# mikkleini/slam.net

Hardware: AMD Instinct MI355X
Metric: candidate-pose distance evals/sec on 2048^2 map, 1080-ray scan, 1/2/4/8 GPU (higher is better)
Workload: dtype f32 transform + u16 gather / integer sum

## Files before the change

include/slamhip.h:

```cpp
#ifndef SLAMHIP_H
#define SLAMHIP_H

#include <stddef.h>
#include <stdint.h>

#ifdef __cplusplus
extern "C" {
#endif

#define SLAMHIP_OK            0
#define SLAMHIP_ERR_INVALID  (-1)
#define SLAMHIP_ERR_HIP      (-2)
#define SLAMHIP_ERR_NOMEM    (-3)
#define SLAMHIP_ERR_STATE    (-4)
#define SLAMHIP_ERR_RCCL     (-5)
#define SLAMHIP_ERR_TIMEOUT  (-6)

typedef struct slamhip_ctx    slamhip_ctx;
typedef struct slamhip_cs     slamhip_cs;
typedef struct slamhip_csproc slamhip_csproc;
typedef struct slamhip_hs     slamhip_hs;
typedef struct slamhip_hsproc slamhip_hsproc;
typedef struct slamhip_group  slamhip_group;
typedef struct slamhip_comm   slamhip_comm;
// ... 69 lines not shown
                                      int32_t count, uint64_t *d_out_key);
int32_t slamhip_cs_search_shard_enqueue(slamhip_cs *cs, const float search_pose[3], int32_t first, int32_t count,
                                        const uint64_t **d_key);
int32_t slamhip_cs_key_read(slamhip_cs *cs, const uint64_t *d_key, uint64_t *out_key);
int32_t slamhip_cs_pose_from_key(slamhip_cs *cs, const float search_pose[3], uint64_t key,
                                 float out_pose[3], int32_t *out_dist, int32_t *out_index);

int32_t slamhip_cs_update_holemap(slamhip_cs *cs, const float pose[3], float hole_width, int32_t quality);
int32_t slamhip_cs_update_holemap_pxcs(slamhip_cs *cs, const float pxcs[4], float hole_width, int32_t quality);
int32_t slamhip_cs_update_obstaclemap(slamhip_cs *cs, const float pose[3], int32_t max_obstacle_hits);
int32_t slamhip_cs_update_obstaclemap_pxcs(slamhip_cs *cs, const float pxcs[4], int32_t max_obstacle_hits);
int32_t slamhip_cs_last_holemap_pixels(slamhip_cs *cs, int64_t *out_pixels);
int32_t slamhip_cs_maps_checksum(slamhip_cs *cs, uint64_t out[2]);

int32_t slamhip_cs_selfcheck_failures(slamhip_cs *cs, uint32_t *out_failures);

int32_t slamhip_cs_prelaunch_stats(slamhip_cs *cs, uint64_t out[4]);

int32_t slamhip_cs_plan_stats(slamhip_cs *cs, uint64_t out[4]);

int32_t slamhip_cs_search_and_update(slamhip_cs *cs, const float search_pose[3], float hole_width,
                                     int32_t quality, int32_t max_obstacle_hits, float out_pose[3],
                                     int32_t *out_dist, int32_t *out_index);
int32_t slamhip_cs_scan_search_and_update(slamhip_cs *cs, const float *xy, int32_t n_points, const float search_pose[3], float hole_width,
                                          int32_t quality, int32_t max_obstacle_hits, float out_pose[3], int32_t *out_dist,
                                          int32_t *out_index);
int32_t slamhip_cs_search_and_update_pxcs(slamhip_cs *cs, const float *pxcs_search, const float *pxcs_update_hole,
                                          const float *pxcs_update_obstacle, int32_t K,
                                          float hole_width, int32_t quality, int32_t max_obstacle_hits,
                                          int32_t *out_index, int32_t *out_dist);
// ... 147 lines not shown
```

slam.net_amd/capi.py:

```python
import ctypes as C
import os
import re

import numpy as np

_HERE = os.path.dirname(os.path.abspath(__file__))
SO_PATH = os.path.join(_HERE, "libslamhip.so")
HEADER = os.path.join(os.path.dirname(_HERE), "include", "slamhip.h")

OK = 0
ERR_INVALID, ERR_HIP, ERR_NOMEM, ERR_STATE, ERR_RCCL, ERR_TIMEOUT = -1, -2, -3, -4, -5, -6
K_CS_PREP, K_CS_DISTANCE, K_CS_REDUCE, K_CS_HOLEMAP, K_CS_OBSTACLE, K_HS_MATCH, K_HS_UPDATE = range(7)

CELL_DTYPE = np.dtype([("update_index", np.int32), ("value", np.float32)])


class MatchReport(C.Structure):
    _fields_ = [("pose_map", C.c_float * 3), ("H", C.c_float * 9), ("dTr", C.c_float * 3), ("residual", C.c_float),
                ("n_in_map", C.c_int32), ("n_points", C.c_int32), ("level", C.c_int32)]


REPORT_DTYPE = np.dtype([("pose_map", np.float32, 3), ("H", np.float32, (3, 3)), ("dTr", np.float32, 3),
                         ("residual", np.float32), ("n_in_map", np.int32), ("n_points", np.int32), ("level", np.int32)])
assert C.sizeof(MatchReport) == REPORT_DTYPE.itemsize == 76
# ... 92 lines not shown
        "slamhip_cs_update_holemap": (i32, [vp, fp, f, i32]),
        "slamhip_cs_update_holemap_pxcs": (i32, [vp, fp, f, i32]),
        "slamhip_cs_update_obstaclemap": (i32, [vp, fp, i32]),
        "slamhip_cs_update_obstaclemap_pxcs": (i32, [vp, fp, i32]),
        "slamhip_cs_last_holemap_pixels": (i32, [vp, P(i64)]),
        "slamhip_cs_maps_checksum": (i32, [vp, P(u64)]),
        "slamhip_cs_search_and_update": (i32, [vp, fp, f, i32, i32, fp, ip, ip]),
        "slamhip_cs_scan_search_and_update": (i32, [vp, fp, i32, fp, f, i32, i32, fp, ip, ip]),
        "slamhip_cs_search_and_update_pxcs": (i32, [vp, fp, fp, fp, i32, f, i32, i32, ip, ip]),
        "slamhip_cs_update_maps_pxcs": (i32, [vp, fp, fp, f, i32, i32]),
        "slamhip_cs_search_report": (i32, [vp, fp, i32, fp, srp]),
        "slamhip_cs_search_distances": (i32, [vp, ip, i32]),
        "slamhip_cs_search_and_update_report": (i32, [vp, fp, i32, f, i32, i32, fp, srp]),
        "slamhip_cs_scan_search_and_update_report": (i32, [vp, fp, i32, fp, i32, f, i32, i32, fp, srp]),
        "slamhip_cs_selfcheck_failures": (i32, [vp, P(C.c_uint32)]),
        "slamhip_cs_prelaunch_stats": (i32, [vp, P(C.c_uint64)]),
        "slamhip_cs_plan_stats": (i32, [vp, P(C.c_uint64)]),
        "slamhip_cs_prepared_lists": (i32, [vp, P(C.c_uint64), P(C.c_uint64)]),
        "slamhip_csproc_create": (i32, [vp, f, i32, i32, fp, f, f, i32, i32, vpp]),
        "slamhip_csproc_destroy": (i32, [vp]),
        "slamhip_csproc_reset": (i32, [vp]),
        "slamhip_csproc_update": (i32, [vp, fp, ip, i32, fp]),
        "slamhip_csproc_get_pose": (i32, [vp, fp]),
        "slamhip_csproc_set_params": (i32, [vp, i32, f, i32, i32, i32]),
        "slamhip_csproc_set_seed": (i32, [vp, u64]),
        "slamhip_csproc_set_lattice": (i32, [vp, i32]),
        "slamhip_csproc_set_offsets": (i32, [vp, fp, i32]),
        "slamhip_csproc_set_search_report": (i32, [vp, i32, i32]),
        "slamhip_csproc_get_report": (i32, [vp, srp, ip]),
        "slamhip_csproc_cs": (i32, [vp, vpp]),
# ... 98 lines not shown
```

slam.net_amd/coreslam.py:

```python
import ctypes as C

import numpy as np

from . import capi


class Context:

    def __init__(self, device=0):
        self._h = C.c_void_p()
        capi.call("slamhip_ctx_create", int(device), C.byref(self._h))

    def close(self):
        if self._h:
            capi.lib().slamhip_ctx_destroy(self._h)
            self._h = C.c_void_p()

    @property
    def stream(self):
        return capi.lib().slamhip_ctx_stream(self._h)

    def synchronize(self):
        capi.call("slamhip_ctx_synchronize", self._h)

# ... 232 lines not shown
        v = (C.c_uint64 * 4)()
        capi.call("slamhip_cs_prelaunch_stats", self._h, v)
        return tuple(int(x) for x in v)

    @property
    def plan_stats(self):
        v = (C.c_uint64 * 4)()
        capi.call("slamhip_cs_plan_stats", self._h, v)
        return tuple(int(x) for x in v)

    @property
    def selfcheck_failures(self):
        v = C.c_uint32()
        capi.call("slamhip_cs_selfcheck_failures", self._h, C.byref(v))
        return v.value

    def search_and_update(self, search_pose, hole_width=0.6, quality=50, max_hits=10):
        sp = capi.f32(search_pose)
        pose = np.empty(3, np.float32); d, i = C.c_int32(), C.c_int32()
        capi.call("slamhip_cs_search_and_update", self._h, capi.fptr(sp), C.c_float(hole_width), int(quality),
                  int(max_hits), capi.fptr(pose), C.byref(d), C.byref(i))
        return pose, d.value, i.value


    def scan_search_and_update(self, xy, search_pose, hole_width=0.6, quality=50, max_hits=10):
        pts = np.ascontiguousarray(xy, np.float32).reshape(-1, 2)
        sp = capi.f32(search_pose)
        pose = np.empty(3, np.float32); d, i = C.c_int32(), C.c_int32()
        capi.call("slamhip_cs_scan_search_and_update", self._h, capi.fptr(pts), int(pts.shape[0]), capi.fptr(sp), C.c_float(hole_width), int(quality),
                  int(max_hits), capi.fptr(pose), C.byref(d), C.byref(i))
# ... 145 lines not shown
```

slam.net_amd/csrc/coreslam.hip:

```cpp
#include "cs_internal.h"
#include "det_trig.h"
#include "obstacle_dev.h"
#include <algorithm>
#include <numeric>
#include <math.h>
#include <stdlib.h>

__global__ void k_fill_u16(uint16_t *p, size_t n, uint16_t v)
{
    size_t i = (size_t)blockIdx.x * blockDim.x + threadIdx.x;
    const size_t stride = (size_t)gridDim.x * blockDim.x;
    for (; i < n; i += stride) p[i] = v;
}

__global__ void k_pack_holemap(const uint16_t *__restrict__ pix, uint8_t *__restrict__ out, size_t n_bytes)
{
    size_t i = (size_t)blockIdx.x * blockDim.x + threadIdx.x;
    if (i >= n_bytes) return;
    out[i] = (uint8_t)(((pix[i * 2] >> 12) << 4) | (pix[i * 2 + 1] >> 12));
}

__device__ static inline void philox4x32_10(uint32_t c[4], uint32_t k0, uint32_t k1)
{
    for (int r = 0; r < 10; r++) {
// ... 1372 lines not shown
extern "C" int32_t slamhip_cs_plan_stats(slamhip_cs *cs, uint64_t out[4])
{
    SH_CHECK_ARG(cs && out);
    for (int k = 0; k < 4; k++) out[k] = cs->plan_stats[k];
    return SLAMHIP_OK;
}

extern "C" int32_t slamhip_cs_selfcheck_failures(slamhip_cs *cs, uint32_t *out)
{
    SH_CHECK_ARG(cs && out);
    SH_HIP(hipSetDevice(cs->ctx->device));
    unsigned int *h = (unsigned int *)(cs->h_key + 8);
    SH_HIP(hipMemcpyAsync(h, cs->d_verify, sizeof(unsigned int) * 8, hipMemcpyDeviceToHost, cs->ctx->stream));
    SH_HIP(hipStreamSynchronize(cs->ctx->stream));
    *out = h[0];
    return SLAMHIP_OK;
}

extern "C" int32_t slamhip_cs_update_maps_pxcs(slamhip_cs *cs, const float pxcs_hole[4], const float pxcs_obstacle[4], float hole_width,
                                               int32_t quality, int32_t max_obstacle_hits)
{
    SH_CHECK_ARG(cs && pxcs_hole && quality >= 0 && quality <= 256 && max_obstacle_hits >= -128 && max_obstacle_hits <= 127);
    SH_HIP(hipSetDevice(cs->ctx->device));
    cs->last_hole_pixels = 0; cs->hole_pixels_pending = false;
    if (cs->n_points <= 0) return SLAMHIP_OK;
    SH_TRY(cs_launch_holemap_update(cs, nullptr, make_float4(pxcs_hole[0], pxcs_hole[1], pxcs_hole[2], pxcs_hole[3]), make_float4(0, 0, 0, 0), hole_width, quality));
    if (pxcs_obstacle)
        SH_TRY(cs_launch_obstacle_update(cs, nullptr, make_float4(pxcs_obstacle[0], pxcs_obstacle[1], pxcs_obstacle[2], pxcs_obstacle[3]), max_obstacle_hits));
    return finish_holemap(cs);
}
// ... 303 lines not shown
```

slam.net_amd/csrc/cs_internal.h:

```cpp
#pragma once
#include "common.h"
#include <time.h>
#include <stdio.h>
#include <stdlib.h>
#include <vector>
#include <utility>

#define CS_RB_MAX 64
#define CS_RB_EXTENT_PX 128.0f
#define K1_GROUP 1024
#define K1_GROUP_BIG 2048
#define K1_RING_SLOTS 4
#define K1_GROUP_SMALL 512
#define K1_PLAN_SLOTS 8


struct k1_block_term { double a, b, m, n, nr; };

struct slamhip_cs {
    slamhip_ctx *ctx;
    float physical;
    int hs; float hscale;
    int os; float oscale;
    uint16_t *d_hole;
    int8_t *d_obst;

    int n_points, cap_points;
    void *d_scan_blob, *h_scan_blob;
    char *d_scan_cur; size_t scan_blob_bytes; int scan_buf;
// ... 178 lines not shown
```

slam.net_amd/csrc/distance.hip:

```cpp
#include "cs_internal.h"
#include "det_trig.h"
#include <stdlib.h>
#include <algorithm>

#define K1_THREADS 256

__device__ static inline void k1_coords(const float4 q, const float2 p, float &fx, float &fy)
{
    fx = q.x + q.z * p.x;  fx = fx - q.w * p.y;
    fy = q.y + q.w * p.x;  fy = fy + q.z * p.y;
}

template <bool SAFE>
__device__ static inline void k1_gather_global(const uint16_t *__restrict__ map, int S, const float4 q, const float2 p,
                                               uint32_t &sum, uint32_t &cnt)
{
    float fx, fy;
    k1_coords(q, p, fx, fy);
    int ix, iy;
    if (SAFE) { ix = sh_f2i(fx); iy = sh_f2i(fy); }
    else      { ix = (int)fx;    iy = (int)fy; }
    const bool ok = ((unsigned)ix < (unsigned)S) & ((unsigned)iy < (unsigned)S);
    uint32_t v = 0;
    if (ok) v = map[(size_t)iy * S + ix];
// ... 105 lines not shown
        }
        __syncthreads();
    }
    if (w == 0) {
        for (int off = 32; off > 0; off >>= 1) {
            const unsigned long long o = __shfl_down(key, off, 64);
            key = o < key ? o : key;
        }
        if (lane == 0 && key != ~0ull) atomicMin(key_out, key);
    }
}

#define K1_KIND_SHARED 1
#define K1_KIND_GLOBAL 2
#define K1_KIND_BAND 3
#define K1_MAXP 16
#define K1_MAXR 512
#define K1_MAXBANDS 4
#define K1_MAXSTEPS (K1_MAXP * K1_MAXBANDS * 2)
static_assert(K1_MAXBANDS == 4, "the step threads split t into (piece, band) with shifts");
#define K1_TABLE_G 64
#define K1_TABLE_WGS 2048
#define K1_MAXCUT 596
#define K1_ACC_INMAP 36
#define K1_ACC_ARRIVED 50
#define K1_ZERO_OFS 0
#define K1_TILE_OFS 16

struct k1_args {
    const uint16_t *map; int S;
// ... 31 lines not shown
        unsigned short nbp;
        unsigned short first, nc;
    } tab[K1_TABLE_G];
    alignas(4) unsigned char wg_pos[K1_TABLE_WGS];
    alignas(4) unsigned short cut[K1_MAXCUT];
};
static_assert(sizeof(k1_args) <= 4096, "kernel arguments are limited to 4 KB");
static_assert(sizeof(k1_args::tab_rec) == 8 && offsetof(k1_args, tab) % 8 == 0, "table records are 8-byte aligned");
#define K1_PLAN_STEPS 15
#define K1_PLAN_REC_WORDS 128

#ifdef K1_TIMES
__device__ unsigned long long g_k1_times[4096 * 16];
__device__ unsigned long long g_k1_wstart[4096 * 16];
__device__ unsigned long long g_k1_sub[4096 * 8];
#define K1_SUB(k, v) { if (threadIdx.x == 0 && blockIdx.x < 4096) g_k1_sub[blockIdx.x * 8 + (k)] += (v); }
#define K1_STAMP(k) { if (threadIdx.x == 0 && blockIdx.x < 4096) g_k1_times[blockIdx.x * 16 + (k)] = wall_clock64(); }
#else
#define K1_STAMP(k) {}
#endif

__device__ static inline unsigned k1_tile_addr(int ix, int iy, int pitch2, int kofs)
{
    unsigned t, a;
    asm("v_lshl_add_u32 %0, %1, 1, %2" : "=v"(t) : "v"(ix), "s"(kofs));
    asm("v_mad_u32_u24 %0, %1, %2, %3" : "=v"(a) : "v"(iy), "s"(pitch2), "v"(t));
    return a;
}
__device__ static inline float k1_den(int v) { return __uint_as_float(v < 0 ? (0x80000000u | (unsigned)(-v)) : (unsigned)v); }
__device__ static inline unsigned k1_tile_addr_d(float fx, float fy, float two_d, float pitch2_d, float c_d)
{
    const float g = fmaf(truncf(fy), pitch2_d, fmaf(truncf(fx), two_d, c_d));
    return __float_as_uint(g);
}
typedef __attribute__((address_space(3))) const uint16_t k1_lds_u16;
__device__ static inline uint32_t k1_lds_load(unsigned addr) { return *(k1_lds_u16 *)(size_t)addr; }
typedef __attribute__((address_space(3))) const float k1_lds_f;
__device__ static inline float2 k1_point_lds(unsigned lds_addr)
{
    k1_lds_f *p = (k1_lds_f *)(size_t)lds_addr;
    return make_float2(p[0], p[1]);
}

typedef float k1_f32x4a8 __attribute__((ext_vector_type(4), aligned(8)));
__device__ static inline float4 k1_points2_lds(unsigned lds_addr)
{
    const k1_f32x4a8 v = *(__attribute__((address_space(3))) const k1_f32x4a8 *)(size_t)lds_addr;
    return make_float4(v.x, v.y, v.z, v.w);
// ... 138 lines not shown

    const uint16_t *__restrict__ map = a.map;
    const int S = a.S, count = a.count;
    const int t = threadIdx.x, lane = t & 63;
    int zv;
    asm volatile("v_mov_b32 %0, 0" : "=v"(zv));
    const int wv = __builtin_amdgcn_readfirstlane(t >> 6);
    const k1_wg_t W = k1_wg_decode(a, (int)blockIdx.x);
    const int g = W.g, nc = W.nc, nbp = W.nbp;
    if (a.ring_reset && blockIdx.x == 0 && t == 0)
        __hip_atomic_store(a.ring_reset, ~0ull, __ATOMIC_RELAXED, __HIP_MEMORY_SCOPE_AGENT);
    if (a.started && blockIdx.x == 0 && t == 0)
        __hip_atomic_store(a.started, a.launch_no, __ATOMIC_RELAXED, __HIP_MEMORY_SCOPE_SYSTEM);
    K1_STAMP(0)
#ifdef K1_TIMES
    if (t == 0 && blockIdx.x < 4096) { for (int k = 0; k < 8; k++) g_k1_sub[blockIdx.x * 8 + k] = 0; }
    if (t == 0 && blockIdx.x < 4096) { for (int k = 10; k < 16; k++) g_k1_times[blockIdx.x * 16 + k] = 0; g_k1_times[blockIdx.x * 16 + 14] = (unsigned long long)g; g_k1_times[blockIdx.x * 16 + 15] = (unsigned long long)nc; }
    if (lane == 0 && blockIdx.x < 4096) g_k1_wstart[blockIdx.x * 16 + (wv & 15)] = wall_clock64();
    if (t == 0 && blockIdx.x < 4096) {
        unsigned hw, xcc;
        asm volatile("s_getreg_b32 %0, hwreg(HW_REG_HW_ID)" : "=s"(hw));
        asm volatile("s_getreg_b32 %0, hwreg(HW_REG_XCC_ID)" : "=s"(xcc));
        g_k1_wstart[blockIdx.x * 16 + 15] = ((unsigned long long)(xcc & 15u) << 16) | ((hw >> 8) & 0xffu);
    }
#endif
    const int bp = W.bp, rlo = W.rlo, rhi = W.rhi;
    const int nrays = rhi - rlo;
    if (a.scan_flag) {
        uint32_t v = 0;
        if (wv == 0) {
            int spins = 0;
// ... 221 lines not shown
            const unsigned long long ts1 = wall_clock64();
            if (s > 0) K1_SUB(0, ts1 - ts0)
#endif
            const int4 ca = *(const int4 *)&stepbuf[s * 8], cb = *(const int4 *)&stepbuf[s * 8 + 4];
            {
                const int sn = s + 1 < nsteps ? s + 1 : s;
                K1_PREFETCH(sn, s + 1 < nsteps)
            }
#ifdef K1_TIMES
            const unsigned long long ts2 = wall_clock64();
            K1_SUB(1, ts2 - ts1) K1_SUB(3, 1ull)
#endif
            const int kind = __builtin_amdgcn_readfirstlane(cb.y);
            const int nr = __builtin_amdgcn_readfirstlane(cb.z) >> 16;
#ifdef K1_TIMES
            if (t == 0 && blockIdx.x < 4096) g_k1_times[blockIdx.x * 16 + 10 + kind] += (unsigned long long)nr;
            if (t == 0 && blockIdx.x < 4096 && s < 3)
                g_k1_sub[blockIdx.x * 8 + 5 + s] = (unsigned long long)kind | ((unsigned long long)__builtin_amdgcn_readfirstlane(ca.z) << 4) | ((unsigned long long)__builtin_amdgcn_readfirstlane(ca.w) << 16) | ((unsigned long long)nr << 32);
#endif
            const unsigned pbase = cpts_lds + (unsigned)zv + (unsigned)(__builtin_amdgcn_readfirstlane(cb.z) & 0xffff) * 8u;
            const int x0a = __builtin_amdgcn_readfirstlane(ca.x), y0 = __builtin_amdgcn_readfirstlane(ca.y);
            const int w8 = __builtin_amdgcn_readfirstlane(ca.z), h = __builtin_amdgcn_readfirstlane(ca.w);
            const int pitch2 = w8 << 1;
            const int kofs = (int)smem_lds + K1_TILE_OFS - ((y0 * w8 + x0a) << 1);
            const unsigned zaddr = smem_lds + K1_ZERO_OFS + (unsigned)zv;
            const bool daddr = !a.noden && (unsigned)S * (unsigned)pitch2 + 2u * (unsigned)S + (1u << 18) < (1u << 23);
            float two_v, p2d_v, cd_v;
            {
                const float two_s = k1_den(2), p2d_s = k1_den(pitch2), cd_s = k1_den(kofs);
                asm volatile("v_mov_b32 %0, %1" : "=v"(two_v) : "s"(two_s));
                asm volatile("v_mov_b32 %0, %1" : "=v"(p2d_v) : "s"(p2d_s));
                asm volatile("v_mov_b32 %0, %1" : "=v"(cd_v) : "s"(cd_s));
            }
            if (K1_EXP == 2 || K1_EXP == 3) { sum[0] += (uint32_t)nr; continue; }
            if (kind != K1_KIND_GLOBAL) {
                const bool checked = kind == K1_KIND_BAND;
                uint32_t va[CPL], vb[CPL];
                int r = 0;
                float4 pn = k1_points2_lds(pbase);
                float2 pa_n = make_float2(pn.x, pn.y), pb_n = make_float2(pn.z, pn.w);
#pragma unroll
                for (int k = 0; k < CPL; k++) { va[k] = k1_lds_load(zaddr); vb[k] = k1_lds_load(zaddr); }
                __builtin_amdgcn_sched_barrier(0);
                if (!checked && daddr) {
#define K1_DPAIR(P, NEXTREAD)                                                                       \
                    {                                                                               \
                        unsigned ada[CPL], adb[CPL];                                                \
                        float cxa_ = 0.f, sya_ = 0.f, sxa_ = 0.f, cya_ = 0.f, cxb_ = 0.f, syb_ = 0.f, sxb_ = 0.f, cyb_ = 0.f; \
                        if (LAT) {                                                                  \
                            cxa_ = q[0].z * (P).x; sya_ = q[0].w * (P).y; sxa_ = q[0].w * (P).x; cya_ = q[0].z * (P).y; \
// ... 107 lines not shown
                        k1_coords(q[k], pa, fx, fy);
                        const int ix = (int)fx, iy = (int)fy;
                        const bool ok = ((unsigned)(ix - x0a) < (unsigned)w8) & ((unsigned)(iy - y0) < (unsigned)h);
                        if (VERIFY) {
                            if (!ok && !checked) atomicAdd(a.verify, 1u);
                            if (ok && map[(size_t)iy * S + ix] != *(const uint16_t *)(smem + (k1_tile_addr(ix, iy, pitch2, kofs) - smem_lds))) atomicAdd(a.verify, 1u);
                        }
                        sum[k] += k1_lds_load(ok ? k1_tile_addr(ix, iy, pitch2, kofs) : zaddr);
                        if (checked) cnt[k] += ok ? 1u : 0u;
                    }
                }
#pragma unroll
                for (int k = 0; k < CPL; k++) sum[k] += va[k] + vb[k];
                if (VERIFY && t == 0) atomicAdd(a.verify + (checked ? 4 : 1), (unsigned)(nr * 4));
            } else {
                int r = 0;
                for (; r + 1 < nr; r += 2) {
                    const float2 pa = k1_point_lds(pbase + r * 8), pb = k1_point_lds(pbase + r * 8 + 8);
                    uint32_t ga[CPL], gb[CPL]; bool oka[CPL], okb[CPL];
#pragma unroll
                    for (int k = 0; k < CPL; k++) {
                        float fxa, fya, fxb, fyb;
                        k1_coords(q[k], pa, fxa, fya);
                        k1_coords(q[k], pb, fxb, fyb);
                        const int ixa = (int)fxa, iya = (int)fya, ixb = (int)fxb, iyb = (int)fyb;
                        oka[k] = ((unsigned)ixa < (unsigned)S) & ((unsigned)iya < (unsigned)S);
                        okb[k] = ((unsigned)ixb < (unsigned)S) & ((unsigned)iyb < (unsigned)S);
                        ga[k] = map[oka[k] ? (size_t)iya * S + ixa : 0];
                        gb[k] = map[okb[k] ? (size_t)iyb * S + ixb : 0];
                    }
#pragma unroll
                    for (int k = 0; k < CPL; k++) {
                        sum[k] += (oka[k] ? ga[k] : 0u) + (okb[k] ? gb[k] : 0u);
                        cnt[k] += (oka[k] ? 1u : 0u) + (okb[k] ? 1u : 0u);
                    }
                }
                if (r < nr) {
                    const float2 pa = k1_point_lds(pbase + r * 8);
#pragma unroll
                    for (int k = 0; k < CPL; k++) k1_gather_global<false>(map, S, q[k], pa, sum[k], cnt[k]);
                }
                if (VERIFY && t == 0) atomicAdd(a.verify + 3, (unsigned)(nr * 4));
            }
#ifdef K1_TIMES
            K1_SUB(2, wall_clock64() - ts2)
#endif
        }
#ifdef K1_TIMES
        K1_SUB(4, clock64() - sclk0)
#endif
#undef K1_PREFETCH
    }
    K1_STAMP(7)

    typedef unsigned long long u64;
    if (K1_EXP == 4) { if (sum[0] == 0x12345u && cnt[0] == 77u) a.verify[0] = 1u; return; }
    u64 *acc = a.acc + (size_t)g * GROUP + (size_t)t;
    u64 tot[CPL];
#pragma unroll
    for (int k = 0; k < CPL; k++) {
// ... 153 lines not shown

static int32_t ensure_partial(slamhip_cs *cs, size_t bytes)
{
    if (bytes <= cs->cap_partial) return SLAMHIP_OK;
    if (cs->d_partial) (void)hipFree(cs->d_partial);
    cs->d_partial = nullptr; cs->cap_partial = 0;
    bytes += bytes / 4;
    SH_HIP(hipMalloc(&cs->d_partial, bytes));
    cs->cap_partial = bytes;
    return SLAMHIP_OK;
}

constexpr int K1_BAND_PARTS = 2;
constexpr float K1_BAND_STAGE = 5.0f;
constexpr double K1_CUT_CAND = 0.9;
constexpr double K1_FBAND = 1.9, K1_FGLOBAL = 3.0;
constexpr double K1_STEPCOST = 8.0;
constexpr double K1_TAILW = 1.5;

static bool k1_chunks_legal(const slamhip_cs *cs, int nc)
{
    const int R = cs->n_points, n_rb = cs->n_rb;
    const int *rb = cs->h_rb_start.data();
    if (nc < 1 || nc > R) return false;
    int b = 0;
    const int dq = R / nc, dr = R % nc;
    int rlo = 0, rem = 0;
    for (int c = 0; c < nc; c++) {
        int rhi = rlo + dq;
        rem += dr;
        if (rem >= nc) { rem -= nc; rhi++; }
// ... 697 lines not shown
            (void)hipMemcpyFromSymbol(sb.data(), HIP_SYMBOL(g_k1_sub), sizeof(unsigned long long) * sb.size());
            double a0 = 0, a1 = 0, a2 = 0, a3 = 0, mhz = 0; int nm_ = 0;
            for (int i = 0; i < nw; i++) {
                a0 += (double)sb[i * 8] * 0.01; a1 += (double)sb[i * 8 + 1] * 0.01; a2 += (double)sb[i * 8 + 2] * 0.01; a3 += (double)sb[i * 8 + 3];
                const double comp = (double)(h[i * 16 + 7] - h[i * 16 + 6]) * 0.01;
                if (comp > 1.0) { mhz += (double)sb[i * 8 + 4] / (comp + (double)(h[i * 16 + 6] - h[i * 16 + 5]) * 0.01); nm_++; }
            }
            fprintf(stderr, "[k1 times] compute phase, mean per WG: steps %.2f | restaging %.2f us | prefetch issue %.2f us | gather loops %.2f us | shader clock ~%.0f MHz (steps incl. first staging)\n",
                    a3 / nw, a0 / nw, a1 / nw, a2 / nw, nm_ ? mhz / nm_ : 0.0);
            for (int oi = 0; oi < nw; oi += nw / 24 > 0 ? nw / 24 : 1) {
                const int i = order[(size_t)oi];
                fprintf(stderr, "  wg %4d g %2d: steps %d restaging %5.2f prefetch %5.2f loops %5.2f | rays shared %d global %d band %d\n", i, (int)h[i * 16 + 14], (int)sb[i * 8 + 3],
                        (double)sb[i * 8] * 0.01, (double)sb[i * 8 + 1] * 0.01, (double)sb[i * 8 + 2] * 0.01, (int)h[i * 16 + 11], (int)h[i * 16 + 12], (int)h[i * 16 + 13]);
            }
        }
        for (int g = 0; g < n_groups; g++) {
            double cs_ = 0, cm = 0; int n = 0; long long k4[4] = { 0, 0, 0, 0 };
            for (int i = 0; i < nw; i++) if ((int)h[i * 16 + 14] == g) {
                const double c = (double)(h[i * 16 + 7] - h[i * 16 + 6]) * 0.01;
                cs_ += c; cm = std::max(cm, c); n++;
                for (int k = 0; k < 4; k++) k4[k] += (long long)h[i * 16 + 10 + k];
            }
            fprintf(stderr, "  group %2d: chunks %2d | ray-steps own %lld shared %lld global %lld band %lld | compute mean %.2f max %.2f us\n",
                    g, n, k4[0], k4[1], k4[2], k4[3], n ? cs_ / n : 0.0, cm);
        }
    }
}
#endif

int32_t cs_launch_distance(slamhip_cs *cs, int mode, const float pose[3], int count, bool want_dist, bool cand_sane,
                           uint64_t *key_dst)
{
    slamhip_ctx *ctx = cs->ctx;
    if (cs->n_points <= 0) SH_FAIL(SLAMHIP_ERR_STATE, "no scan set (slamhip_cs_set_scan)");
    cs->rep_dist_valid = false;
    SH_TRY(cs_flush_scan(cs));
    cs->k1_launch_no = cs->launch_count;
    static const int force_global = (int)sh_env_int("SLAMHIP_K1_GLOBAL", 0);
// ... 236 lines not shown
```

slam.net_amd/csrc/k1_pieces.inc:

```
    for (int p = wv; p < npieces; p += NW) {
        const int2 pi = pieces[p];
        const float2 pt = cpts[K1_PIECE_RAY(pi.x + (lane < pi.y ? lane : pi.y - 1))];
        const float4 b0 = *(const float4 *)&bnd[0], b1 = *(const float4 *)&bnd[4];
        const float bb8[8] = { b0.x, b0.y, b0.z, b0.w, b1.x, b1.y, b1.z, b1.w };
        int bx0, by0, bx1, by1;
        k1_ray_box(bb8, pt, bx0, by0, bx1, by1);
        bx0 = k1_wave_red<false>(bx0); by0 = k1_wave_red<false>(by0);
        bx1 = k1_wave_red<true>(bx1);  by1 = k1_wave_red<true>(by1);
        K1_PIECE_STAMP
        struct k1_plan_t { int nsteps, kind, x0a, y0, w8, h, shift; float cost; };
        auto k1_plan = [&](const int4 bx, const int nr_, const int band) -> k1_plan_t {
            k1_plan_t P; P.nsteps = 1; P.kind = K1_KIND_GLOBAL; P.x0a = 0; P.y0 = 0; P.w8 = 8; P.h = 0; P.shift = 0; P.cost = 4.5f * (float)nr_;
            const int cx0 = max(bx.x, 0), cy0 = max(bx.y, 0), cx1 = min(bx.z, S - 1), cy1 = min(bx.w, S - 1);
            if (cx1 < cx0 || cy1 < cy0) { P.nsteps = 0; P.cost = 0.0f; return P; }
            int xa = cx0 & ~7, ww = ((cx1 - xa + 1) + 7) & ~7;
            const int H = cy1 - cy0 + 1;
            if (GROUP >= 1024 && !(ww & 8) && !a.nopad && ww < 512 && (xa + ww + 8 <= S || xa >= 8)) {
                const int wp = ww + 8, vp = wp >> 3, vu = ww >> 3;
                const int shp = 32 - __clz(vp - 1), shu = vu <= 1 ? 0 : 32 - __clz(vu - 1);
                const int hp = min(k1_div(a.budget, wp * 2), PF * NW * (64 >> (shp & 31))), hu = min(k1_div(a.budget, ww * 2), PF * NW * (64 >> (shu & 31)));
                if (hp >= 1 && hu >= 1 && k1_div(H + hp - 1, hp) == k1_div(H + hu - 1, hu)) { if (xa + ww + 8 <= S) ww += 8; else { xa -= 8; ww += 8; } }
            }
            const int vpr = ww >> 3;
            const int sh = vpr <= 1 ? 0 : 32 - __clz(vpr - 1);
            const int hmax = min(k1_div(a.budget, ww * 2), PF * NW * (64 >> (sh & 31)));
            const int nb_ = hmax >= 1 ? k1_div(H + hmax - 1, hmax) : K1_MAXBANDS + 1;
            const bool bands_pay = nb_ == 1 || (float)nb_ * (a.band_stage + 1.9f * (float)nr_) < 4.5f * (float)nr_;
            if (vpr <= 64 && hmax >= 1 && nb_ <= K1_MAXBANDS && bands_pay) {
                P.nsteps = nb_;
                const int hb = k1_div(H + nb_ - 1, nb_);
                const bool whole = nb_ == 1 && cx0 == bx.x && cy0 == bx.y && cx1 == bx.z && cy1 == bx.w;
                P.kind = whole ? K1_KIND_SHARED : K1_KIND_BAND;
                P.x0a = xa; P.w8 = ww; P.shift = sh;
                P.y0 = cy0 + band * hb;
                P.h = min(hb, cy1 + 1 - P.y0);
                const float stage = (float)nb_ * 6.0f + 20.0f * (float)(ww * 2) * (float)H / (float)a.budget;
                P.cost = stage * (2.0f / (float)CPL) + (whole ? (float)nr_ : 1.9f * (float)nb_ * (float)nr_);
                if (P.h <= 0 && band < nb_) P.h = 0;
            }
            return P;
        };
        const int pc = p;
        const int nr_all = pieces[pc].y, r_first = pieces[pc].x;
        const bool planner = lane >= 64 - K1_MAXBANDS;
        const int4 bx = make_int4(bx0, by0, bx1, by1);
        k1_plan_t full = k1_plan(bx, nr_all, planner ? lane - (64 - K1_MAXBANDS) : 0);
        const bool want = GROUP >= 1024 && planner && lane == 63 && !a.nosplit && nr_all >= 8 && full.nsteps != 0 && full.nsteps > 1;
        bool split = false;
        k1_plan_t half;
        half.nsteps = 0; half.kind = K1_KIND_GLOBAL; half.x0a = 0; half.y0 = 0; half.w8 = 8; half.h = 0; half.shift = 0; half.cost = 0.0f;
        int h_first = r_first, h_nr = nr_all;
        if (__builtin_amdgcn_ballot_w64(want) != 0) {
// ... 3 lines not shown
            const bool inA = lane < h1;
            const int A0 = k1_wave_red<false>(inA ? ax0 : 0x7fffffff), A1 = k1_wave_red<false>(inA ? ay0 : 0x7fffffff);
            const int A2 = k1_wave_red<true>(inA ? ax1 : (int)0x80000000), A3 = k1_wave_red<true>(inA ? ay1 : (int)0x80000000);
            const int B0 = k1_wave_red<false>(inA ? 0x7fffffff : ax0), B1 = k1_wave_red<false>(inA ? 0x7fffffff : ay0);
            const int B2 = k1_wave_red<true>(inA ? (int)0x80000000 : ax1), B3 = k1_wave_red<true>(inA ? (int)0x80000000 : ay1);
            const int idx = lane - (64 - 2 * K1_MAXBANDS);
            const int hb_ = idx >= K1_MAXBANDS ? 1 : 0, band_ = idx >= 0 ? idx - hb_ * K1_MAXBANDS : 0;
            const k1_plan_t pa = k1_plan(make_int4(A0, A1, A2, A3), h1, hb_ == 0 ? band_ : 0);
            const k1_plan_t pb = k1_plan(make_int4(B0, B1, B2, B3), nr_all - h1, hb_ == 1 ? band_ : 0);
            split = pa.cost + pb.cost < full.cost;
            half = hb_ ? pb : pa;
            h_first = hb_ ? r_first + h1 : r_first; h_nr = hb_ ? nr_all - h1 : h1;
            if (split) {
                if (idx < 0) continue;
                const int band = band_;
                if (band < half.nsteps && (half.kind == K1_KIND_GLOBAL || half.h > 0) && (half.kind == K1_KIND_BAND ? (nbp == 2 ? (band & 1) == bp : band % nbp == bp) : bp == 0)) {
                    int4 *dst = (int4 *)&stepbuf[K1_STEP_SLOT(atomicAdd(&s_nsteps, 1)) * 8];
                    dst[0] = make_int4(half.x0a, half.y0, half.w8, half.h);
                    dst[1] = make_int4(half.shift, half.kind, h_first | (h_nr << 16), 0);
                }
                continue;
            }
        }
        if (!planner) continue;
        {
            const int band = lane - (64 - K1_MAXBANDS);
            const int prec = r_first | (nr_all << 16);
            const bool live = full.kind == K1_KIND_GLOBAL ? true : full.h > 0;
            if (band < full.nsteps && live && (full.kind == K1_KIND_BAND ? (nbp == 2 ? (band & 1) == bp : band % nbp == bp) : bp == 0)) {
                int4 *dst = (int4 *)&stepbuf[K1_STEP_SLOT(atomicAdd(&s_nsteps, 1)) * 8];
                dst[0] = make_int4(full.x0a, full.y0, full.w8, full.h);
                dst[1] = make_int4(full.shift, full.kind, prec, 0);
            }
        }
    }
```

Measured before the change: 1.074 billion.

## Add bounds-free global gather path for pieces whose ray box lies inside map

The planner now marks a global-gather piece as GLOBAL_IN when its clipped bounding box equals the unclipped one, meaning every sample is inside the map. For such pieces the gather loop skips per-sample bounds checks and counts, computes byte offsets with a float FMA or v_mad_u32_u24, and software-pipelines point loads and gathers across two register sets with scheduling barriers. The general global path is rewritten the same way with its checks kept. This adds code size and register pressure, and correctness depends on the box test covering every sample.

```diff
diff --git a/include/slamhip.h b/include/slamhip.h
--- a/include/slamhip.h
+++ b/include/slamhip.h
@@ -107,6 +107,7 @@
 int32_t slamhip_cs_maps_checksum(slamhip_cs *cs, uint64_t out[2]);
 
 int32_t slamhip_cs_selfcheck_failures(slamhip_cs *cs, uint32_t *out_failures);
+int32_t slamhip_cs_selfcheck_counts(slamhip_cs *cs, uint32_t out[8]);
 
 int32_t slamhip_cs_prelaunch_stats(slamhip_cs *cs, uint64_t out[4]);
 
diff --git a/slam.net_amd/capi.py b/slam.net_amd/capi.py
--- a/slam.net_amd/capi.py
+++ b/slam.net_amd/capi.py
@@ -130,6 +130,7 @@
         "slamhip_cs_search_and_update_report": (i32, [vp, fp, i32, f, i32, i32, fp, srp]),
         "slamhip_cs_scan_search_and_update_report": (i32, [vp, fp, i32, fp, i32, f, i32, i32, fp, srp]),
         "slamhip_cs_selfcheck_failures": (i32, [vp, P(C.c_uint32)]),
+        "slamhip_cs_selfcheck_counts": (i32, [vp, P(C.c_uint32)]),
         "slamhip_cs_prelaunch_stats": (i32, [vp, P(C.c_uint64)]),
         "slamhip_cs_plan_stats": (i32, [vp, P(C.c_uint64)]),
         "slamhip_cs_prepared_lists": (i32, [vp, P(C.c_uint64), P(C.c_uint64)]),
diff --git a/slam.net_amd/coreslam.py b/slam.net_amd/coreslam.py
--- a/slam.net_amd/coreslam.py
+++ b/slam.net_amd/coreslam.py
@@ -270,6 +270,12 @@
         v = C.c_uint32()
         capi.call("slamhip_cs_selfcheck_failures", self._h, C.byref(v))
         return v.value
+
+    @property
+    def selfcheck_counts(self):
+        v = (C.c_uint32 * 8)()
+        capi.call("slamhip_cs_selfcheck_counts", self._h, v)
+        return tuple(int(x) for x in v)
 
     def search_and_update(self, search_pose, hole_width=0.6, quality=50, max_hits=10):
         sp = capi.f32(search_pose)
diff --git a/slam.net_amd/csrc/coreslam.hip b/slam.net_amd/csrc/coreslam.hip
--- a/slam.net_amd/csrc/coreslam.hip
+++ b/slam.net_amd/csrc/coreslam.hip
@@ -1410,6 +1410,17 @@
     SH_HIP(hipMemcpyAsync(h, cs->d_verify, sizeof(unsigned int) * 8, hipMemcpyDeviceToHost, cs->ctx->stream));
     SH_HIP(hipStreamSynchronize(cs->ctx->stream));
     *out = h[0];
+    return SLAMHIP_OK;
+}
+
+extern "C" int32_t slamhip_cs_selfcheck_counts(slamhip_cs *cs, uint32_t out[8])
+{
+    SH_CHECK_ARG(cs && out);
+    SH_HIP(hipSetDevice(cs->ctx->device));
+    unsigned int *h = (unsigned int *)(cs->h_key + 8);
+    SH_HIP(hipMemcpyAsync(h, cs->d_verify, sizeof(unsigned int) * 8, hipMemcpyDeviceToHost, cs->ctx->stream));
+    SH_HIP(hipStreamSynchronize(cs->ctx->stream));
+    for (int k = 0; k < 8; k++) out[k] = h[k];
     return SLAMHIP_OK;
 }
 
diff --git a/slam.net_amd/csrc/cs_internal.h b/slam.net_amd/csrc/cs_internal.h
--- a/slam.net_amd/csrc/cs_internal.h
+++ b/slam.net_amd/csrc/cs_internal.h
@@ -13,6 +13,9 @@
 #define K1_RING_SLOTS 4
 #define K1_GROUP_SMALL 512
 #define K1_PLAN_SLOTS 8
+#define K1_RAYCOST_BAND 1.9f
+#define K1_RAYCOST_GLOBAL 4.5f
+#define K1_RAYCOST_GLOBAL_IN 4.5f
 
 
 struct k1_block_term { double a, b, m, n, nr; };
diff --git a/slam.net_amd/csrc/distance.hip b/slam.net_amd/csrc/distance.hip
--- a/slam.net_amd/csrc/distance.hip
+++ b/slam.net_amd/csrc/distance.hip
@@ -143,6 +143,7 @@
 #define K1_KIND_SHARED 1
 #define K1_KIND_GLOBAL 2
 #define K1_KIND_BAND 3
+#define K1_KIND_GLOBAL_IN 4
 #define K1_MAXP 16
 #define K1_MAXR 512
 #define K1_MAXBANDS 4
@@ -204,6 +205,7 @@
 __device__ unsigned long long g_k1_times[4096 * 16];
 __device__ unsigned long long g_k1_wstart[4096 * 16];
 __device__ unsigned long long g_k1_sub[4096 * 8];
+__device__ unsigned long long g_k1_kind[4096 * 8];
 #define K1_SUB(k, v) { if (threadIdx.x == 0 && blockIdx.x < 4096) g_k1_sub[blockIdx.x * 8 + (k)] += (v); }
 #define K1_STAMP(k) { if (threadIdx.x == 0 && blockIdx.x < 4096) g_k1_times[blockIdx.x * 16 + (k)] = wall_clock64(); }
 #else
@@ -222,6 +224,22 @@
 {
     const float g = fmaf(truncf(fy), pitch2_d, fmaf(truncf(fx), two_d, c_d));
     return __float_as_uint(g);
+}
+__device__ static inline unsigned k1_map_ofs(int ix, int iy, unsigned S2)
+{
+    unsigned a;
+    const unsigned t = (unsigned)ix << 1;
+    asm("v_mad_u32_u24 %0, %1, %2, %3" : "=v"(a) : "v"(iy), "s"(S2), "v"(t));
+    return a;
+}
+__device__ static inline unsigned k1_map_ofs_d(float fx, float fy, float two_d, float s2_d)
+{
+    return __float_as_uint(fmaf(truncf(fy), s2_d, truncf(fx) * two_d));
+}
+__device__ static inline uint32_t k1_map_load(const uint16_t *__restrict__ map, unsigned ofs)
+{
+    asm("" : "+v"(ofs));
+    return *(const uint16_t *)((const char *)map + ofs);
 }
 typedef __attribute__((address_space(3))) const uint16_t k1_lds_u16;
 __device__ static inline uint32_t k1_lds_load(unsigned addr) { return *(k1_lds_u16 *)(size_t)addr; }
@@ -390,7 +408,7 @@
         __hip_atomic_store(a.started, a.launch_no, __ATOMIC_RELAXED, __HIP_MEMORY_SCOPE_SYSTEM);
     K1_STAMP(0)
 #ifdef K1_TIMES
-    if (t == 0 && blockIdx.x < 4096) { for (int k = 0; k < 8; k++) g_k1_sub[blockIdx.x * 8 + k] = 0; }
+    if (t == 0 && blockIdx.x < 4096) { for (int k = 0; k < 8; k++) { g_k1_sub[blockIdx.x * 8 + k] = 0; g_k1_kind[blockIdx.x * 8 + k] = 0; } }
     if (t == 0 && blockIdx.x < 4096) { for (int k = 10; k < 16; k++) g_k1_times[blockIdx.x * 16 + k] = 0; g_k1_times[blockIdx.x * 16 + 14] = (unsigned long long)g; g_k1_times[blockIdx.x * 16 + 15] = (unsigned long long)nc; }
     if (lane == 0 && blockIdx.x < 4096) g_k1_wstart[blockIdx.x * 16 + (wv & 15)] = wall_clock64();
     if (t == 0 && blockIdx.x < 4096) {
@@ -642,7 +660,7 @@
             const int kind = __builtin_amdgcn_readfirstlane(cb.y);
             const int nr = __builtin_amdgcn_readfirstlane(cb.z) >> 16;
 #ifdef K1_TIMES
-            if (t == 0 && blockIdx.x < 4096) g_k1_times[blockIdx.x * 16 + 10 + kind] += (unsigned long long)nr;
+            if (t == 0 && blockIdx.x < 4096) g_k1_times[blockIdx.x * 16 + 10 + (kind == K1_KIND_GLOBAL_IN ? 0 : kind)] += (unsigned long long)nr;
             if (t == 0 && blockIdx.x < 4096 && s < 3)
                 g_k1_sub[blockIdx.x * 8 + 5 + s] = (unsigned long long)kind | ((unsigned long long)__builtin_amdgcn_readfirstlane(ca.z) << 4) | ((unsigned long long)__builtin_amdgcn_readfirstlane(ca.w) << 16) | ((unsigned long long)nr << 32);
 #endif
@@ -661,7 +679,7 @@
                 asm volatile("v_mov_b32 %0, %1" : "=v"(cd_v) : "s"(cd_s));
             }
             if (K1_EXP == 2 || K1_EXP == 3) { sum[0] += (uint32_t)nr; continue; }
-            if (kind != K1_KIND_GLOBAL) {
+            if (kind != K1_KIND_GLOBAL && kind != K1_KIND_GLOBAL_IN) {
                 const bool checked = kind == K1_KIND_BAND;
                 uint32_t va[CPL], vb[CPL];
                 int r = 0;
@@ -799,36 +817,111 @@
                 for (int k = 0; k < CPL; k++) sum[k] += va[k] + vb[k];
                 if (VERIFY && t == 0) atomicAdd(a.verify + (checked ? 4 : 1), (unsigned)(nr * 4));
             } else {
-                int r = 0;
-                for (; r + 1 < nr; r += 2) {
-                    const float2 pa = k1_point_lds(pbase + r * 8), pb = k1_point_lds(pbase + r * 8 + 8);
-                    uint32_t ga[CPL], gb[CPL]; bool oka[CPL], okb[CPL];
-#pragma unroll
-                    for (int k = 0; k < CPL; k++) {
-                        float fxa, fya, fxb, fyb;
-                        k1_coords(q[k], pa, fxa, fya);
-                        k1_coords(q[k], pb, fxb, fyb);
-                        const int ixa = (int)fxa, iya = (int)fya, ixb = (int)fxb, iyb = (int)fyb;
-                        oka[k] = ((unsigned)ixa < (unsigned)S) & ((unsigned)iya < (unsigned)S);
-                        okb[k] = ((unsigned)ixb < (unsigned)S) & ((unsigned)iyb < (unsigned)S);
-                        ga[k] = map[oka[k] ? (size_t)iya * S + ixa : 0];
-                        gb[k] = map[okb[k] ? (size_t)iyb * S + ixb : 0];
-                    }
-#pragma unroll
-                    for (int k = 0; k < CPL; k++) {
-                        sum[k] += (oka[k] ? ga[k] : 0u) + (okb[k] ? gb[k] : 0u);
-                        cnt[k] += (oka[k] ? 1u : 0u) + (okb[k] ? 1u : 0u);
-                    }
+                const bool gin = kind == K1_KIND_GLOBAL_IN;
+                constexpr bool TWO = CPL <= 2;
+                const unsigned S2 = (unsigned)S * 2u;
+                const bool gden = gin && !a.noden && (unsigned)S <= 2048u;
+                float s2d_v;
+                { const float s2d_s = k1_den((int)S2); asm volatile("v_mov_b32 %0, %1" : "=v"(s2d_v) : "s"(s2d_s)); }
+                const int np = nr >> 1;
+                uint32_t gA[2 * CPL], gB[2 * CPL], go[CPL];
+                bool okA[2 * CPL], okB[2 * CPL], oko[CPL];
+#pragma unroll
+                for (int k = 0; k < 2 * CPL; k++) { gA[k] = 0u; gB[k] = 0u; okA[k] = false; okB[k] = false; }
+#pragma unroll
+                for (int k = 0; k < CPL; k++) { go[k] = 0u; oko[k] = false; }
+#define K1_GODD                                                                                     \
+                if (nr & 1) {                                                                        \
+                    const float2 pl = k1_point_lds(pbase + (nr - 1) * 8);                            \
+                    unsigned oo[CPL];                                                                \
+                    _Pragma("unroll") for (int k = 0; k < CPL; k++) {                                \
+                        float fx, fy;                                                                \
+                        k1_coords(q[k], pl, fx, fy);                                                 \
+                        const int ix = (int)fx, iy = (int)fy;                                        \
+                        const bool ok = ((unsigned)ix < (unsigned)S) & ((unsigned)iy < (unsigned)S); \
+                        if (VERIFY && gin && !ok) atomicAdd(a.verify, 1u);                           \
+                        oko[k] = gin && !VERIFY ? true : ok;                                         \
+                        oo[k] = oko[k] ? k1_map_ofs(ix, iy, S2) : 0u;                                \
+                        if (!gin) cnt[k] += ok ? 1u : 0u;                                            \
+                    }                                                                                \
+                    _Pragma("unroll") for (int k = 0; k < CPL; k++) go[k] = k1_map_load(map, oo[k]); \
+                }                                                                                   
+                if (TWO) K1_GODD
+                float4 pn = k1_points2_lds(pbase);
+#define K1_GSTEP(FORM, NEXT, G, OKG)                                                                \
+                {                                                                                   \
+                    const float4 P = pn;                                                            \
+                    pn = k1_points2_lds(pbase + (NEXT) * 16);                                       \
+                    unsigned oa[CPL], ob[CPL]; bool ta[CPL], tb[CPL];                               \
+                    _Pragma("unroll") for (int k = 0; k < CPL; k++) {                               \
+                        float fxa, fya, fxb, fyb;                                                   \
+                        k1_coords(q[k], make_float2(P.x, P.y), fxa, fya);                           \
+                        k1_coords(q[k], make_float2(P.z, P.w), fxb, fyb);                           \
+                        ta[k] = true; tb[k] = true;                                                 \
+                        if ((FORM) == 0) {                                                          \
+                            oa[k] = k1_map_ofs_d(fxa, fya, two_v, s2d_v);                           \
+                            ob[k] = k1_map_ofs_d(fxb, fyb, two_v, s2d_v);                           \
+                        } else {                                                                    \
+                            const int ixa = (int)fxa, iya = (int)fya, ixb = (int)fxb, iyb = (int)fyb; \
+                            oa[k] = k1_map_ofs(ixa, iya, S2);                                       \
+                            ob[k] = k1_map_ofs(ixb, iyb, S2);                                       \
+                            if ((FORM) == 2) {                                                      \
+                                ta[k] = ((unsigned)ixa < (unsigned)S) & ((unsigned)iya < (unsigned)S); \
+                                tb[k] = ((unsigned)ixb < (unsigned)S) & ((unsigned)iyb < (unsigned)S); \
+                                oa[k] = ta[k] ? oa[k] : 0u;                                         \
+                                ob[k] = tb[k] ? ob[k] : 0u;                                         \
+                                cnt[k] += (ta[k] ? 1u : 0u) + (tb[k] ? 1u : 0u);                    \
+                            }                                                                       \
+                        }                                                                           \
+                        if (VERIFY && (FORM) != 2) {                                                \
+                            const int ixa = (int)fxa, iya = (int)fya, ixb = (int)fxb, iyb = (int)fyb; \
+                            if ((unsigned)ixa >= (unsigned)S || (unsigned)iya >= (unsigned)S || (unsigned)ixb >= (unsigned)S || (unsigned)iyb >= (unsigned)S) \
+                                { atomicAdd(a.verify, 1u); oa[k] = 0u; ob[k] = 0u; }    \
+                            else if (oa[k] != ((unsigned)iya * (unsigned)S + (unsigned)ixa) * 2u || ob[k] != ((unsigned)iyb * (unsigned)S + (unsigned)ixb) * 2u) \
+                                atomicAdd(a.verify, 1u);            \
+                        }                                                                           \
+                    }                                                                               \
+                    __builtin_amdgcn_sched_barrier(0);                                              \
+                    if ((FORM) == 2) {                                                              \
+                        _Pragma("unroll") for (int k = 0; k < CPL; k++) sum[k] += (OKG[2 * k] ? G[2 * k] : 0u) + (OKG[2 * k + 1] ? G[2 * k + 1] : 0u); \
+                        _Pragma("unroll") for (int k = 0; k < CPL; k++) { OKG[2 * k] = ta[k]; OKG[2 * k + 1] = tb[k]; } \
+                    } else {                                                                        \
+                        _Pragma("unroll") for (int k = 0; k < CPL; k++) sum[k] += G[2 * k] + G[2 * k + 1]; \
+                    }                                                                               \
+                    _Pragma("unroll") for (int k = 0; k < CPL; k++) { G[2 * k] = k1_map_load(map, oa[k]); G[2 * k + 1] = k1_map_load(map, ob[k]); } \
+                    __builtin_amdgcn_sched_barrier(0);                                              \
                 }
-                if (r < nr) {
-                    const float2 pa = k1_point_lds(pbase + r * 8);
-#pragma unroll
-                    for (int k = 0; k < CPL; k++) k1_gather_global<false>(map, S, q[k], pa, sum[k], cnt[k]);
+#define K1_GLOOP(FORM)                                                                              \
+                {                                                                                   \
+                    int i = 0;                                                                      \
+                    if (TWO) {                                                                      \
+                        for (; i + 1 < np; i += 2) { K1_GSTEP(FORM, i + 1, gA, okA) K1_GSTEP(FORM, i + 2, gB, okB) } \
+                        if (i < np) K1_GSTEP(FORM, i + 1, gA, okA)                                  \
+                    } else {                                                                        \
+                        for (; i < np; i++) K1_GSTEP(FORM, i + 1, gA, okA)                          \
+                    }                                                                               \
                 }
-                if (VERIFY && t == 0) atomicAdd(a.verify + 3, (unsigned)(nr * 4));
+                if (gden) K1_GLOOP(0)
+                else if (gin) K1_GLOOP(1)
+                else K1_GLOOP(2)
+                if (!TWO) K1_GODD
+#undef K1_GLOOP
+#undef K1_GSTEP
+#undef K1_GODD
+                if (gin) {
+#pragma unroll
+                    for (int k = 0; k < CPL; k++) sum[k] += gA[2 * k] + gA[2 * k + 1] + (TWO ? gB[2 * k] + gB[2 * k + 1] : 0u) + go[k];
+                    cnt_all += (uint32_t)nr;
+                } else {
+#pragma unroll
+                    for (int k = 0; k < CPL; k++)
+                        sum[k] += (okA[2 * k] ? gA[2 * k] : 0u) + (okA[2 * k + 1] ? gA[2 * k + 1] : 0u) +
+                                  (TWO ? (okB[2 * k] ? gB[2 * k] : 0u) + (okB[2 * k + 1] ? gB[2 * k + 1] : 0u) : 0u) + (oko[k] ? go[k] : 0u);
+                }
+                if (VERIFY && t == 0) atomicAdd(a.verify + (gin ? 7 : 3), (unsigned)(nr * 4));
             }
 #ifdef K1_TIMES
-            K1_SUB(2, wall_clock64() - ts2)
+            { const unsigned long long tl_ = wall_clock64() - ts2; K1_SUB(2, tl_) if (t == 0 && blockIdx.x < 4096) g_k1_kind[blockIdx.x * 8 + (kind == K1_KIND_GLOBAL_IN ? 0 : kind)] += tl_; }
 #endif
         }
 #ifdef K1_TIMES
@@ -1012,7 +1105,8 @@
 constexpr int K1_BAND_PARTS = 2;
 constexpr float K1_BAND_STAGE = 5.0f;
 constexpr double K1_CUT_CAND = 0.9;
-constexpr double K1_FBAND = 1.9, K1_FGLOBAL = 3.0;
+constexpr double K1_FBAND = (double)K1_RAYCOST_BAND;
+constexpr double K1_FGLOBAL = 3.0;
 constexpr double K1_STEPCOST = 8.0;
 constexpr double K1_TAILW = 1.5;
 
@@ -1740,6 +1834,16 @@
                         (double)sb[i * 8] * 0.01, (double)sb[i * 8 + 1] * 0.01, (double)sb[i * 8 + 2] * 0.01, (int)h[i * 16 + 11], (int)h[i * 16 + 12], (int)h[i * 16 + 13]);
             }
         }
+        {
+            std::vector<unsigned long long> kk((size_t)nw * 8);
+            (void)hipMemcpyFromSymbol(kk.data(), HIP_SYMBOL(g_k1_kind), sizeof(unsigned long long) * kk.size());
+            static const char *kn[4] = { "global_in", "shared", "global", "band" };
+            double tk[4] = { 0, 0, 0, 0 }, rk[4] = { 0, 0, 0, 0 };
+            for (int i = 0; i < nw; i++) for (int k = 0; k < 4; k++) { tk[k] += (double)kk[(size_t)i * 8 + k] * 10.0; rk[k] += (double)h[(size_t)i * 16 + 10 + k]; }
+            fprintf(stderr, "[k1 times] gather loops, ns per ray and workgroup:");
+            for (int k = 0; k < 4; k++) fprintf(stderr, " %s %.1f (%.0f rays) |", kn[k], rk[k] > 0 ? tk[k] / rk[k] : 0.0, rk[k]);
+            fprintf(stderr, "\n");
+        }
         for (int g = 0; g < n_groups; g++) {
             double cs_ = 0, cm = 0; int n = 0; long long k4[4] = { 0, 0, 0, 0 };
             for (int i = 0; i < nw; i++) if ((int)h[i * 16 + 14] == g) {
@@ -1747,7 +1851,7 @@
                 cs_ += c; cm = std::max(cm, c); n++;
                 for (int k = 0; k < 4; k++) k4[k] += (long long)h[i * 16 + 10 + k];
             }
-            fprintf(stderr, "  group %2d: chunks %2d | ray-steps own %lld shared %lld global %lld band %lld | compute mean %.2f max %.2f us\n",
+            fprintf(stderr, "  group %2d: chunks %2d | ray-steps global_in %lld shared %lld global %lld band %lld | compute mean %.2f max %.2f us\n",
                     g, n, k4[0], k4[1], k4[2], k4[3], n ? cs_ / n : 0.0, cm);
         }
     }
diff --git a/slam.net_amd/csrc/k1_pieces.inc b/slam.net_amd/csrc/k1_pieces.inc
--- a/slam.net_amd/csrc/k1_pieces.inc
+++ b/slam.net_amd/csrc/k1_pieces.inc
@@ -10,8 +10,10 @@
         K1_PIECE_STAMP
         struct k1_plan_t { int nsteps, kind, x0a, y0, w8, h, shift; float cost; };
         auto k1_plan = [&](const int4 bx, const int nr_, const int band) -> k1_plan_t {
-            k1_plan_t P; P.nsteps = 1; P.kind = K1_KIND_GLOBAL; P.x0a = 0; P.y0 = 0; P.w8 = 8; P.h = 0; P.shift = 0; P.cost = 4.5f * (float)nr_;
             const int cx0 = max(bx.x, 0), cy0 = max(bx.y, 0), cx1 = min(bx.z, S - 1), cy1 = min(bx.w, S - 1);
+            const bool inside = cx0 == bx.x && cy0 == bx.y && cx1 == bx.z && cy1 == bx.w;
+            const float gcost = inside ? K1_RAYCOST_GLOBAL_IN : K1_RAYCOST_GLOBAL;
+            k1_plan_t P; P.nsteps = 1; P.kind = inside ? K1_KIND_GLOBAL_IN : K1_KIND_GLOBAL; P.x0a = 0; P.y0 = 0; P.w8 = 8; P.h = 0; P.shift = 0; P.cost = gcost * (float)nr_;
             if (cx1 < cx0 || cy1 < cy0) { P.nsteps = 0; P.cost = 0.0f; return P; }
             int xa = cx0 & ~7, ww = ((cx1 - xa + 1) + 7) & ~7;
             const int H = cy1 - cy0 + 1;
@@ -25,7 +27,7 @@
             const int sh = vpr <= 1 ? 0 : 32 - __clz(vpr - 1);
             const int hmax = min(k1_div(a.budget, ww * 2), PF * NW * (64 >> (sh & 31)));
             const int nb_ = hmax >= 1 ? k1_div(H + hmax - 1, hmax) : K1_MAXBANDS + 1;
-            const bool bands_pay = nb_ == 1 || (float)nb_ * (a.band_stage + 1.9f * (float)nr_) < 4.5f * (float)nr_;
+            const bool bands_pay = nb_ == 1 || (float)nb_ * (a.band_stage + K1_RAYCOST_BAND * (float)nr_) < gcost * (float)nr_;
             if (vpr <= 64 && hmax >= 1 && nb_ <= K1_MAXBANDS && bands_pay) {
                 P.nsteps = nb_;
                 const int hb = k1_div(H + nb_ - 1, nb_);
@@ -35,7 +37,7 @@
                 P.y0 = cy0 + band * hb;
                 P.h = min(hb, cy1 + 1 - P.y0);
                 const float stage = (float)nb_ * 6.0f + 20.0f * (float)(ww * 2) * (float)H / (float)a.budget;
-                P.cost = stage * (2.0f / (float)CPL) + (whole ? (float)nr_ : 1.9f * (float)nb_ * (float)nr_);
+                P.cost = stage * (2.0f / (float)CPL) + (whole ? (float)nr_ : K1_RAYCOST_BAND * (float)nb_ * (float)nr_);
                 if (P.h <= 0 && band < nb_) P.h = 0;
             }
             return P;
@@ -69,7 +71,7 @@
             if (split) {
                 if (idx < 0) continue;
                 const int band = band_;
-                if (band < half.nsteps && (half.kind == K1_KIND_GLOBAL || half.h > 0) && (half.kind == K1_KIND_BAND ? (nbp == 2 ? (band & 1) == bp : band % nbp == bp) : bp == 0)) {
+                if (band < half.nsteps && (half.kind == K1_KIND_GLOBAL || half.kind == K1_KIND_GLOBAL_IN || half.h > 0) && (half.kind == K1_KIND_BAND ? (nbp == 2 ? (band & 1) == bp : band % nbp == bp) : bp == 0)) {
                     int4 *dst = (int4 *)&stepbuf[K1_STEP_SLOT(atomicAdd(&s_nsteps, 1)) * 8];
                     dst[0] = make_int4(half.x0a, half.y0, half.w8, half.h);
                     dst[1] = make_int4(half.shift, half.kind, h_first | (h_nr << 16), 0);
@@ -81,7 +83,7 @@
         {
             const int band = lane - (64 - K1_MAXBANDS);
             const int prec = r_first | (nr_all << 16);
-            const bool live = full.kind == K1_KIND_GLOBAL ? true : full.h > 0;
+            const bool live = full.kind == K1_KIND_GLOBAL || full.kind == K1_KIND_GLOBAL_IN ? true : full.h > 0;
             if (band < full.nsteps && live && (full.kind == K1_KIND_BAND ? (nbp == 2 ? (band & 1) == bp : band % nbp == bp) : bp == 0)) {
                 int4 *dst = (int4 *)&stepbuf[K1_STEP_SLOT(atomicAdd(&s_nsteps, 1)) * 8];
                 dst[0] = make_int4(full.x0a, full.y0, full.w8, full.h);
```

Measured after the change: 956.3 million. 0.891x the previous value.
